# lfeng-nl/paddle-operator

Hardware: AMD Instinct MI355X
Metric: launched tokens/sec (GPT-2-medium PaddleJob through the pdo operator, collective DP over RCCL) (higher is better)
Workload: dtype bf16; 1 GPU; model=gpt2-medium, global_batch=64, micro_batch_per_gpu=64, seq_len=1024, parallelism=dp1, pod_layout=1x1, grad_reduce=bf16, buckets=2, ops=hip, device=AMD Radeon Graphics

## Files before the change

### csrc/hip/bind.cpp

```cpp
#include <c10/hip/HIPStream.h>
#include <torch/extension.h>

#include <cmath>

#include "kernels.h"

namespace {

using pdo::bf16;

hipStream_t cur_stream() { return c10::hip::getCurrentHIPStream().stream(); }

#define CHECK_DEV(t) TORCH_CHECK((t).is_cuda(), #t " must be a GPU tensor")
#define CHECK_CONTIG(t) TORCH_CHECK((t).is_contiguous(), #t " must be contiguous")
#define CHECK_BF16(t) TORCH_CHECK((t).scalar_type() == at::kBFloat16, #t " must be bf16")
#define CHECK_F32(t) TORCH_CHECK((t).scalar_type() == at::kFloat, #t " must be float32")
#define CHECK_I64(t) TORCH_CHECK((t).scalar_type() == at::kLong, #t " must be int64")
#define CHECK_IN(t) \
  CHECK_DEV(t);     \
  CHECK_CONTIG(t)
#define CHECK_RC(rc, what) TORCH_CHECK((rc) == 0, what " rejected the shape (code ", rc, ")")

inline bf16* bp(const at::Tensor& t) { return reinterpret_cast<bf16*>(t.data_ptr()); }
inline float* fp(const at::Tensor& t) { return t.data_ptr<float>(); }
// ... 324 lines not shown
                           cur_stream()), "adamw_flat");
}

void sgd_flat(at::Tensor w, at::Tensor g, at::Tensor buf, at::Tensor decay, double lr, double mom, double wd,
              double grad_scale) {
  CHECK_IN(w); CHECK_IN(g); CHECK_IN(buf); CHECK_IN(decay);
  CHECK_F32(w); CHECK_F32(g); CHECK_F32(buf); CHECK_F32(decay);
  const long long n = w.numel();
  TORCH_CHECK(g.numel() == n && buf.numel() == n && n % 1024 == 0 && decay.numel() == n / 1024);
  CHECK_RC(pdo::sgd_flat(fp(w), fp(g), fp(buf), fp(decay), n, (float)lr, (float)mom, (float)wd, (float)grad_scale,
                         cur_stream()), "sgd_flat");
}

void splitk_add(at::Tensor part, at::Tensor out, bool accumulate) {
  CHECK_IN(part); CHECK_BF16(part); CHECK_BF16(out);
  TORCH_CHECK(out.is_contiguous() && part.size(0) >= 1 && part[0].numel() == out.numel());
  CHECK_RC(pdo::splitk_add(bp(part), (int)part.size(0), out.numel(), bp(out), accumulate ? 1 : 0, cur_stream()),
           "splitk_add");
}

bool gemm_dw(at::Tensor dy, at::Tensor x, at::Tensor out, bool accumulate, int64_t splits) {
  CHECK_IN(dy); CHECK_IN(x); CHECK_IN(out); CHECK_BF16(dy); CHECK_BF16(x); CHECK_BF16(out);
  TORCH_CHECK(dy.dim() == 2 && x.dim() == 2 && dy.size(0) == x.size(0));
  const long long T = dy.size(0);
  const int M = dy.size(1), N = x.size(1);
  TORCH_CHECK(out.numel() == (int64_t)M * N, "gemm_dw: out must hold M·N elements");
  int s = pdo::gemm_dw_splits(T, M, N);
  if (s == 0) return false;
  if (splits > 0) s = (int)splits;
  at::Tensor ws;
  if (s > 1) ws = at::empty({(int64_t)s * M * N}, dy.options());
  CHECK_RC(pdo::gemm_dw(bp(dy), bp(x), T, M, N, M, N, bp(out), N, accumulate ? 1 : 0, s > 1 ? bp(ws) : nullptr, s,
                        cur_stream()), "gemm_dw");
  return true;
}

void transpose_batched(at::Tensor src, at::Tensor dst, at::Tensor table, at::Tensor host, int64_t tiles) {
  CHECK_IN(src); CHECK_IN(dst); CHECK_IN(table); CHECK_BF16(src); CHECK_BF16(dst);
  TORCH_CHECK(table.scalar_type() == at::kLong && table.dim() == 2 && table.size(1) == 5, "table: int64 [n, 5]");
  TORCH_CHECK(!host.is_cuda() && host.scalar_type() == at::kLong && host.is_contiguous() &&
              host.sizes() == table.sizes(), "transpose_batched: host table must mirror the device table");
  const at::Tensor& t = host;
  const int64_t* e = t.data_ptr<int64_t>();
  int64_t want = 0;
  for (int64_t i = 0; i < t.size(0); ++i, e += 5) {
    TORCH_CHECK(e[0] == want && e[3] % 64 == 0 && e[4] % 64 == 0 && e[3] > 0 && e[4] > 0, "transpose_batched: bad entry ", i);
    TORCH_CHECK(e[1] >= 0 && e[1] + e[3] * e[4] <= src.numel() && e[2] >= 0 && e[2] + e[3] * e[4] <= dst.numel(),
                "transpose_batched: entry ", i, " out of range");
    want += (e[3] / 64) * (e[4] / 64);
  }
  TORCH_CHECK(want == tiles, "transpose_batched: tile count mismatch");
  CHECK_RC(pdo::transpose_bf16_batched(bp(src), bp(dst), reinterpret_cast<const long long*>(table.data_ptr<int64_t>()), (int)table.size(0), tiles,
                                       cur_stream()), "transpose_batched");
}

bool gemm_nt_supported(int64_t M, int64_t N, int64_t K) {
  return M < (1LL << 31) && N < (1LL << 31) && pdo::gemm_nt_ok((int)M, (int)N, (int)K, (int)K, (int)K, (int)N);
}

static void nt_check(const at::Tensor& a, const at::Tensor& b) {
  CHECK_IN(a); CHECK_IN(b); CHECK_BF16(a); CHECK_BF16(b);
  TORCH_CHECK(a.dim() == 2 && b.dim() == 2 && a.size(1) == b.size(1), "gemm_nt: a [M, K], b [N, K]");
  TORCH_CHECK(gemm_nt_supported(a.size(0), b.size(0), a.size(1)), "gemm_nt: M, N % 256 and K % 64 required");
}

at::Tensor gemm_nt(at::Tensor a, at::Tensor b, c10::optional<at::Tensor> bias, c10::optional<at::Tensor> out) {
// ... 859 lines not shown
        py::arg("eps"), py::arg("rbias") = py::none(), py::arg("thr") = 0, py::arg("seed") = 0, py::arg("site") = 0,
        py::arg("step") = 0, py::arg("offset") = 0);
  m.def("layernorm_bwd", &layernorm_bwd, py::arg("dy"), py::arg("x"), py::arg("w"), py::arg("mean"),
        py::arg("rstd"), py::arg("grads") = py::none());
  m.def("layernorm_bwd_add", &layernorm_bwd_add, py::arg("dy"), py::arg("h"), py::arg("w"), py::arg("mean"),
        py::arg("rstd"), py::arg("dres"), py::arg("rbias"), py::arg("grads") = py::none(), py::arg("thr") = 0,
        py::arg("seed") = 0, py::arg("site") = 0, py::arg("step") = 0, py::arg("offset") = 0,
        py::arg("want_dx") = true);
  m.def("bias_gelu_fwd", &bias_gelu_fwd);
  m.def("bias_gelu_bwd", &bias_gelu_bwd, py::arg("dy"), py::arg("x"), py::arg("b"), py::arg("db_out") = py::none());
  m.def("bias_grad", &bias_grad, py::arg("dy"), py::arg("out") = py::none());
  m.def("xent_fwd", &xent_fwd);
  m.def("xent_bwd", &xent_bwd);
  m.def("xent_fused", &xent_fused);
  m.def("embed_fwd", &embed_fwd, py::arg("idx"), py::arg("wte"), py::arg("wpe"), py::arg("thr") = 0,
        py::arg("seed") = 0, py::arg("site") = 0, py::arg("step") = 0, py::arg("offset") = 0);
  m.def("embed_bwd", &embed_bwd);
  m.def("embed_bwd_sorted", &embed_bwd_sorted);
  m.def("sumsq", &sumsq);
  m.def("sumsq_chunks", &sumsq_chunks);
  m.def("set_adamw_variant", [](int v) { pdo::adamw_set_variant(v); });
  m.def("sumsq_total", &sumsq_total);
  m.def("adamw_flat", &adamw_flat);
  m.def("sgd_flat", &sgd_flat);
  m.def("splitk_add", &splitk_add);
  m.def("transpose", &transpose, py::arg("x"), py::arg("out") = py::none());
  m.def("transpose_batched", &transpose_batched);
  m.def("colsum_defer", &colsum_defer);
  m.def("colsum_flush", &colsum_flush);
  m.def("colsum_pending", &colsum_pending);
  m.def("axpy_dev_", &axpy_dev_);
  m.def("gemm_dw", &gemm_dw, py::arg("dy"), py::arg("x"), py::arg("out"), py::arg("accumulate") = true,
        py::arg("splits") = 0);
  m.def("gemm_dw_splits", &pdo::gemm_dw_splits);
  m.def("gemm_nt_supported", &gemm_nt_supported);
  m.def("gemm_nt_stats", &gemm_nt_stats);
  m.def("gemm_nt_stats_rows", [](int64_t K) { return pdo::gemm_nt_stats_rows((int)K); });
  m.def("gemm_nt_epi_ok", [](int64_t M, int64_t N, int64_t K) {
    return M < (1LL << 31) && N < (1LL << 31) && pdo::gemm_nt_epi_ok((int)M, (int)N, (int)K) != 0;
  });
  m.def("gemm_dw_impl", [](int impl) {
    const int prev = pdo::gemm_dw_get_impl();
    if (impl >= 0) pdo::gemm_dw_set_impl(impl);
    return prev;
  }, py::arg("impl") = -1, "select gemm_dw's mainloop (0 = 8-wave, 1.. = 4-wave variants); returns the previous");
  m.def("gemm_nt_impl", [](int impl) {
    const int prev = pdo::gemm_nt_get_impl();
    if (impl >= 0) pdo::gemm_nt_set_impl(impl);
    return prev;
  }, py::arg("impl") = -1, "select gemm_nt's mainloop (0 = 8-wave ring, 1 = 4-wave); returns the previous");
  m.def("gemm_nt4_dynamic", [](int on) {
    static int cur = 0;
    const int prev = cur;
    if (on >= 0) pdo::gemm_nt4_set_dynamic(cur = on);
    return prev;
  }, py::arg("on") = -1, "gemm_nt4 tile order: 1 = dynamic per-XCD counters, 0 = static (default); returns the previous");
  m.def("gemm_nt", &gemm_nt, py::arg("a"), py::arg("b"), py::arg("bias") = py::none(), py::arg("out") = py::none());
  m.def("gemm_nt_gelu", &gemm_nt_gelu, py::arg("a"), py::arg("b"), py::arg("bias"), py::arg("saved_grad") = false);
  m.def("gemm_nt_dgelu", &gemm_nt_dgelu, py::arg("a"), py::arg("b"), py::arg("pre"), py::arg("bias"),
        py::arg("db_out") = py::none(), py::arg("saved_grad") = false);
  m.def("bn_act_fwd", &bn_act_fwd);
  m.def("bn_act_bwd_pair", &bn_act_bwd_pair);
  m.def("bn_act_fwd_tiles_bnres", &bn_act_fwd_tiles_bnres);
  m.def("bn_act_fwd_tiles", &bn_act_fwd_tiles);
  m.def("conv_ok", &conv_ok);
  m.def("conv_fwd", &conv_fwd, py::arg("x"), py::arg("w"), py::arg("stride"), py::arg("pad"),
// ... 51 lines not shown
```

### csrc/hip/gemm_dw4.hip

```cpp
#include <type_traits>

#include "dw_tile.h"
#include "kernels.h"

namespace pdo {

namespace {

constexpr int BM = 256, BN = 256, BK = 64;
constexpr int LROW = 256;
constexpr int TILE = BK * LROW;
constexpr int OPB = TILE * 2;
constexpr int NTHR = 256;
using Tile = DwTile<LROW>;

__global__ __launch_bounds__(NTHR, 1) void gemm_dw4_kernel(const bf16* __restrict__ A, const bf16* __restrict__ B,
                                                           int lda, int ldb, int M, int N, int ksteps_total,
                                                           int splits, bf16* __restrict__ C, int ldc,
                                                           long long split_stride, int accumulate) {
  __shared__ __attribute__((aligned(16))) bf16 smem[2 * 2 * TILE];
  const int tid = threadIdx.x, lane = tid & 63;
  const int w = __builtin_amdgcn_readfirstlane(tid >> 6);
  const int wm = w >> 1, wn = w & 1;
  const int tiles_n = N / BN, tiles_m = (M + BM - 1) / BM;
// ... 152 lines not shown
        const int m = m0 + wm * 128 + 32 * mb + (r & 3) + 8 * (r >> 2) + 4 * hh;
        if (m >= M) continue;
        const int n = n0 + wn * 128 + 32 * nb + li;
        bf16* p = Cb + (size_t)m * ldc + n;
        float x = v[r];
        if (accumulate) x += (float)*p;
        *p = (bf16)x;
      }
    }
}

__device__ __forceinline__ int swz16(int r) { return ((r & 3) | ((((r >> 2) ^ (r >> 3)) & 1) << 2)) << 1; }
__device__ __forceinline__ int loff16(int r, int ch) { return r * LROW + ((ch ^ swz16(r)) << 3); }
__device__ __forceinline__ int frag_base16(int cb, int lane) {
  const int g = lane >> 4, t = lane & 15, q = t >> 2, p = t & 3;
  const int col = cb + 4 * p;
  return loff16(4 * g + q, col >> 3) + (col & 7);
}
template <int K0>
__device__ __forceinline__ bf16x8 frag16(const bf16* T) {
  return ld_tr8(T + K0 * LROW, T + (K0 + 16) * LROW);
}

struct DwGather {
  const bf16* x;
  unsigned xbytes;
  int C, S, IH, IW, TA, TB;
  int TC;
  float inv_TA, inv_TB;
  int st, pad;
  float* part;
};

template <bool GATHER>
__global__ __launch_bounds__(NTHR, 1) void gemm_dw4m16_kernel(const bf16* __restrict__ A, const bf16* __restrict__ B,
                                                              int lda, int ldb, int M, int N, int ksteps_total,
                                                              int splits, bf16* __restrict__ C, int ldc,
                                                              long long split_stride, int accumulate,
                                                              const DwGather gx) {
  __shared__ __attribute__((aligned(16))) bf16 smem[2 * 2 * TILE];
  const int tid = threadIdx.x, lane = tid & 63;
  const int w = __builtin_amdgcn_readfirstlane(tid >> 6);
  const int wm = w >> 1, wn = w & 1;
  const int tiles_n = N / BN, tiles_m = (M + BM - 1) / BM;
  const int nwg = tiles_m * tiles_n * splits;
  const int id = xcd_remap((int)blockIdx.x, nwg);
  const int tn = id % tiles_n;
  const int tm = (id / tiles_n) % tiles_m;
  const int split = id / (tiles_n * tiles_m);
  const int pq = (ksteps_total >> 1) / splits, pr = (ksteps_total >> 1) % splits;
  const int k0 = 2 * (split * pq + min(split, pr));
  const int nk = 2 * (pq + (split < pr ? 1 : 0));
  const int m0 = tm * BM, n0 = tn * BN;

  const int rl = lane >> 5, rw = 2 * w + rl;
  unsigned voffA[2], voffB[2];
#pragma unroll
  for (int par = 0; par < 2; ++par) {
    const int cs = (lane & 31) ^ swz16(8 * par + rw);
    const int csa = (m0 + BM > M && cs >= 16) ? cs - 16 : cs;
    voffA[par] = (unsigned)((rl * lda + csa * 8) * 2);
    voffB[par] = (unsigned)((rl * ldb + cs * 8) * 2);
  }
  const bf16* baseA = A + ((size_t)k0 * BK + 2 * w) * lda + m0;
  const bf16* baseB = GATHER ? A : B + ((size_t)k0 * BK + 2 * w) * ldb + n0;
  const unsigned stepAb = (unsigned)(16 * lda), stepBb = (unsigned)(16 * ldb);
  const unsigned lds0 = lds_addr(smem) + (unsigned)(w * 1024);
  int gdh[2] = {0, 0}, gdw[2] = {0, 0}, gci[2] = {0, 0};
  const __amdgpu_buffer_rsrc_t rsX = buf_rsrc(GATHER ? gx.x : A, GATHER ? (int)gx.xbytes : 0);
  if constexpr (GATHER) {
#pragma unroll
    for (int par = 0; par < 2; ++par) {
      const int col = n0 + (((lane & 31) ^ swz16(8 * par + rw)) << 3);
      const int tap = col / gx.C, r = tap / gx.S;
      gci[par] = col - tap * gx.C;
      gdh[par] = col < gx.TC ? r - gx.pad : -(1 << 20);
      gdw[par] = tap - r * gx.S - gx.pad;
    }
  }
  struct Src {
    const char* a;
    const char* b;
    unsigned sa, sb;
    int kt;
  };
// ... 42 lines not shown
  bf16x8 f0[16], f1[16];

  {
    const Src s0 = srcs(0), s1 = srcs(1);
#pragma unroll
    for (int p = 0; p < 16; ++p) dma(s0, B0{}, p);
#pragma unroll
    for (int p = 0; p < 16; ++p) dma(s1, B1{}, p);
  }
  vm_wait<16>();
  __builtin_amdgcn_sched_barrier(0);
  __builtin_amdgcn_s_barrier();
  __builtin_amdgcn_sched_barrier(0);
#pragma unroll
  for (int q = 0; q < 16; ++q) f0[q] = rd(B0{}, 0, q);
  auto tileH = [&](int t, auto buf_tag, auto more_tag, auto first_tag, auto eout_tag) {
    constexpr int BUF = decltype(buf_tag)::value;
    constexpr bool MORE = decltype(more_tag)::value;
    constexpr bool FIRST = decltype(first_tag)::value;
    constexpr bool EOUT = decltype(eout_tag)::value;
    using NB = std::integral_constant<int, BUF ^ 1>;
    using SB = std::integral_constant<int, BUF>;
    Src sn2{};
    if constexpr (EOUT) sn2 = srcs(t + 2);
    asm volatile("s_waitcnt lgkmcnt(0)" ::: "memory");
    __builtin_amdgcn_sched_barrier(0);
    __builtin_amdgcn_s_barrier();
    __builtin_amdgcn_sched_barrier(0);
#pragma unroll
    for (int g = 0; g < 16; ++g) {
      const int mb = g >> 1, nb0 = 4 * (g & 1);
#pragma unroll
      for (int u = 0; u < 4; ++u) {
        if (FIRST) mfma16_acc0(acc[mb][nb0 + u], f0[mb], f0[8 + nb0 + u]);
        else mfma16_acc(acc[mb][nb0 + u], f0[mb], f0[8 + nb0 + u]);
      }
      f1[g] = rd(buf_tag, 1, g);
      if constexpr (EOUT) {
        if (g & 1) dma(sn2, SB{}, (g >> 1) < 4 ? (g >> 1) : (g >> 1) + 4);
      }
      __builtin_amdgcn_sched_barrier(0);
    }
    if constexpr (MORE || EOUT) {
      if constexpr (EOUT)
        asm volatile("s_waitcnt vmcnt(8) lgkmcnt(0)" ::: "memory");
      else
        asm volatile("s_waitcnt vmcnt(0) lgkmcnt(0)" ::: "memory");
      __builtin_amdgcn_sched_barrier(0);
      __builtin_amdgcn_s_barrier();
      __builtin_amdgcn_sched_barrier(0);
    }
#pragma unroll
    for (int g = 0; g < 16; ++g) {
      const int mb = g >> 1, nb0 = 4 * (g & 1);
#pragma unroll
      for (int u = 0; u < 4; ++u) mfma16_acc(acc[mb][nb0 + u], f1[mb], f1[8 + nb0 + u]);
      if constexpr (MORE) f0[g] = rd(NB{}, 0, g);
      if constexpr (EOUT) {
        if (g & 1) dma(sn2, SB{}, (g >> 1) < 4 ? (g >> 1) + 4 : (g >> 1) + 8);
      }
      __builtin_amdgcn_sched_barrier(0);
    }
  };
  using T_ = std::true_type;
  using F_ = std::false_type;
  tileH(0, B0{}, T_{}, T_{}, T_{});
  tileH(1, B1{}, T_{}, F_{}, T_{});
  for (int t = 2; t < nk - 2; t += 2) {
    tileH(t, B0{}, T_{}, F_{}, T_{});
    tileH(t + 1, B1{}, T_{}, F_{}, T_{});
  }
  tileH(nk - 2, B0{}, T_{}, F_{}, F_{});
  tileH(nk - 1, B1{}, F_{}, F_{}, F_{});

  asm volatile("s_nop 7\n\ts_nop 7" ::: "memory");
  bf16* Cb = C + (size_t)split * split_stride;
  const int g4 = lane >> 4, li = lane & 15;
  if (m0 + wm * 128 >= M) return;
  if constexpr (GATHER) {
    float* P = gx.part + (size_t)split * split_stride;
#pragma unroll
    for (int mb = 0; mb < 8; ++mb)
#pragma unroll
      for (int nb = 0; nb < 8; ++nb) {
        float v[4];
#pragma unroll
        for (int r = 0; r < 4; ++r) asm volatile("v_accvgpr_read_b32 %0, %1" : "=v"(v[r]) : "a"(acc[mb][nb][r]));
#pragma unroll
        for (int r = 0; r < 4; ++r) {
          const int m = m0 + wm * 128 + 16 * mb + 4 * g4 + r;
          P[(size_t)m * ldc + n0 + wn * 128 + 16 * nb + li] = v[r];
        }
      }
    return;
  }
#pragma unroll
  for (int mb = 0; mb < 8; ++mb)
#pragma unroll
    for (int nb = 0; nb < 8; ++nb) {
      float v[4];
#pragma unroll
      for (int r = 0; r < 4; ++r) asm volatile("v_accvgpr_read_b32 %0, %1" : "=v"(v[r]) : "a"(acc[mb][nb][r]));
#pragma unroll
      for (int r = 0; r < 4; ++r) {
        const int m = m0 + wm * 128 + 16 * mb + 4 * g4 + r;
        bf16* p = Cb + (size_t)m * ldc + n0 + wn * 128 + 16 * nb + li;
        float x = v[r];
        if (accumulate) x += (float)*p;
        *p = (bf16)x;
      }
    }
}

}

int gemm_dw4(const bf16* A, const bf16* B, long long T, int M, int N, int lda, int ldb, bf16* C, int ldc,
             int accumulate, bf16* ws, int splits, hipStream_t st, int variant) {
  if (M % (BM / 2) || N % BN || T % BK || splits < 1 || splits > 16) return -2;
  const long long ks = T / BK;
  if (ks > 0x7fffffffLL) return -2;
  if (ks % 2 || (ks / 2) / splits < 2) return -2;
  const int tiles = ((M + BM - 1) / BM) * (N / BN);
  const int grid = tiles * splits;
  bf16* out = C;
  int ldo = ldc;
  long long stride = 0;
  int acc = accumulate;
  if (splits > 1) {
    if (!ws || ldc != N) return -3;
    out = ws;
    ldo = N;
    stride = (long long)M * N;
    acc = 0;
  }
  if (variant == 1)
    gemm_dw4_kernel<<<grid, NTHR, 0, st>>>(A, B, lda, ldb, M, N, (int)ks, splits, out, ldo, stride, acc);
  else
    gemm_dw4m16_kernel<false><<<grid, NTHR, 0, st>>>(A, B, lda, ldb, M, N, (int)ks, splits, out, ldo, stride, acc,
                                                     DwGather{});
  if (splits > 1) return splitk_add(ws, splits, (long long)M * N, C, accumulate, st);
  return 0;
}

int conv_wgrad_dw4_splits(int Kout, int TC, long long M) {
  const long long tiles = (long long)((Kout + 255) / 256) * ((TC + 255) / 256);
  const long long pairs = M / 128;
  static const int ncu = [] {
    int dev = 0, n = 0;
    if (hipGetDevice(&dev) != hipSuccess || hipDeviceGetAttribute(&n, hipDeviceAttributeMultiprocessorCount, dev) != hipSuccess)
      n = 256;
    return n > 0 ? n : 256;
  }();
  long long sp = ncu / tiles;
  if (sp > pairs / 2) sp = pairs / 2;
  if (sp > 256) sp = 256;
  return sp < 1 ? 1 : (int)sp;
}

int conv_wgrad_dw4(const bf16* dy, const bf16* x, int N, int H, int W, int C, int Kout, int R, int S, int stride,
                   int pad, float* part, int splits, hipStream_t st) {
  const int Ho = (H + 2 * pad - R) / stride + 1, Wo = (W + 2 * pad - S) / stride + 1;
  const long long M = (long long)N * Ho * Wo;
  const int TC = R * S * C, TCp = (TC + BN - 1) / BN * BN;
  if (Kout % (BM / 2) || C % 8 || M % (2 * BK) || M >= (1LL << 31)) return -2;
  const long long ks = M / BK;
  if (splits < 1 || (ks / 2) / splits < 2) return -2;
  if ((long long)N * H * W * C * 2 >= (1LL << 31)) return -2;
  DwGather g{x, (unsigned)((long long)N * H * W * C * 2), C, S, H, W, Ho, Wo, TC, 1.f / (float)Ho, 1.f / (float)Wo,
             stride, pad, part};
  const int grid = ((Kout + BM - 1) / BM) * (TCp / BN) * splits;
  gemm_dw4m16_kernel<true><<<grid, NTHR, 0, st>>>(dy, nullptr, Kout, 0, Kout, TCp, (int)ks, splits, nullptr, TCp,
                                                  (long long)Kout * TCp, 0, g);
  return 0;
}

}
```

### csrc/hip/kernels.h

```cpp
#pragma once
#include <hip/hip_runtime.h>
#include <stdint.h>

#include "philox.h"

namespace pdo {
typedef __bf16 bf16;

struct ColOut {
  bf16* p[3] = {nullptr, nullptr, nullptr};
  int seg = 1 << 30;
  int acc = 0;
  static ColOut one(bf16* o, int C) {
    ColOut c;
    c.p[0] = o;
    c.seg = C;
    return c;
  }
};

int layernorm_fwd(const bf16* x, const bf16* r, const bf16* rb, const bf16* w, const bf16* b, bf16* h, bf16* y,
                  float* mean, float* rstd, int N, int C, float eps, hipStream_t st,
                  const DropArgs* drop = nullptr);
int layernorm_bwd_grid(int N);
// ... 68 lines not shown
                       float* ss, const float* rtile_part, int rG, int rtile_rows, const bf16* r, const float* rw,
                       const float* rb, float* rrunning_mean, float* rrunning_var, float reps, float rmomentum,
                       float* rmean, float* rinvstd, float* rss, long long M, int C, int relu, bf16* y,
                       unsigned char* mask, hipStream_t st, float* merge = nullptr);
int bn_fwd_scratch_floats(long long M, int C);
int bn_bwd_scratch_pair_floats(long long M, int C);
int bn_bwd_pair(const bf16* dy, const unsigned char* mask, const bf16* x, const float* mean, const float* invstd,
                const float* w, float* dw, float* db, int accumulate, const bf16* r, const float* rmean,
                const float* rinvstd, const float* rw, float* rdw, float* rdb, int raccumulate, long long M, int C,
                bf16* dx, bf16* dr, float* scratch, hipStream_t st);
int bn_relu_pool_fwd_tiles(const float* tile_part, int G, int tile_rows, const bf16* x, const float* w, const float* b,
                           float* running_mean, float* running_var, int N, int H, int W, int C, float eps,
                           float momentum, bf16* y, uint8_t* arg, bf16* xsel, float* mean, float* invstd, float* ss,
                           hipStream_t st, float* merge = nullptr);
int pool_bn_bwd_scratch_floats(int N, int H, int W, int C);
int pool_bn_bwd(const bf16* dy, const bf16* y, const bf16* xsel, const uint8_t* arg, const bf16* x, const float* mean,
                const float* invstd, const float* w, const float* b, int N, int H, int W, int C, bf16* dx, float* dw,
                float* db, int accumulate, float* scratch, hipStream_t st);
int bn_fwd(const bf16* x, const bf16* res, const float* w, const float* b, float* running_mean, float* running_var,
           long long M, int C, float eps, float momentum, int relu, bf16* y, float* mean, float* invstd,
           float* scratch, hipStream_t st, unsigned char* mask = nullptr);
int bn_bwd_scratch_floats(long long M, int C);
int bn_bwd(const bf16* dy, const bf16* y, const bf16* x, const float* mean, const float* invstd, const float* w,
           const float* b, long long M, int C, int relu, bf16* dx, bf16* dres, float* dw, float* db, int accumulate,
           float* scratch, hipStream_t st);
int maxpool3s2_fwd(const bf16* x, int N, int H, int W, int C, bf16* y, uint8_t* arg, hipStream_t st);
int maxpool3s2_bwd(const bf16* dy, const uint8_t* arg, int N, int H, int W, int C, bf16* dx, hipStream_t st);
int gap_bwd(const bf16* dy, int N, int HW, int C, bf16* dx, hipStream_t st);
int gemm_dw_splits(long long T, int M, int N);
int gemm_dw(const bf16* A, const bf16* B, long long T, int M, int N, int lda, int ldb, bf16* C, int ldc,
            int accumulate, bf16* ws, int splits, hipStream_t st);
int gemm_dw4(const bf16* A, const bf16* B, long long T, int M, int N, int lda, int ldb, bf16* C, int ldc,
             int accumulate, bf16* ws, int splits, hipStream_t st, int variant);
void gemm_dw_set_impl(int impl);
int gemm_dw_get_impl();
int gemm_nt_ok(int M, int N, int K, int lda, int ldb, int ldc);
int gemm_nt_epi_ok(int M, int N, int K);
int gemm_nt_stats_rows(int K);
int gemm_nt_dbias_rows(int M, int K);
int gemm_nt(const bf16* A, const bf16* B, int M, int N, int K, int lda, int ldb, bf16* C, int ldc, int epi,
            const bf16* bias, bf16* Y, int ldy, float* dbias_part, hipStream_t st);
int gemm_nt4(const bf16* A, const bf16* B, int M, int N, int K, int lda, int ldb, bf16* C, int ldc, int epi,
             const bf16* bias, bf16* Y, int ldy, float* dbias_part, hipStream_t st);
void gemm_nt_set_impl(int impl);
void gemm_nt4_set_dynamic(int on);
int gemm_nt_get_impl();
int transpose_bf16(const bf16* in, bf16* out, int R, int C, hipStream_t st);
int transpose_bf16_batched(const bf16* src, bf16* dst, const long long* table, int n, long long tiles,
                           hipStream_t st);
int splitk_add(const bf16* part, int s, long long n, bf16* out, int accumulate, hipStream_t st);

int bias_gelu_fwd(const bf16* x, const bf16* b, bf16* y, long long N, int F, hipStream_t st);
int bias_gelu_bwd_groups(long long N, int F);
int bias_gelu_bwd(const bf16* dy, const bf16* x, const bf16* b, bf16* dx, float* part, float* scratch, bf16* db,
                  long long N, int F, hipStream_t st, int accumulate = 0);

int xent_fwd(const bf16* logits, const int64_t* tgt, float* row_loss, float* lse, float* stats, int N, int Vp, int V,
             hipStream_t st);
int xent_fused(bf16* logits, const int64_t* tgt, const float* inv_cnt, float* row_loss, float* loss, int N, int Vp,
               int V, hipStream_t st);
int xent_bwd(const bf16* logits, const int64_t* tgt, const float* lse, const float* dloss, const float* stats,
             bf16* dlogits, int N, int Vp, int V, hipStream_t st);

int embed_fwd(const int64_t* idx, const bf16* wte, const bf16* wpe, bf16* y, int B, int S, int C, hipStream_t st,
              const DropArgs* drop = nullptr);
int embed_bwd(const bf16* dy, const int64_t* idx, float* acc, bf16* dwte, bf16* dwpe, int B, int S, int C, int Vp,
// ... 41 lines not shown
```

### paddle_operator_amd/ops/__init__.py

```python
from .core import (
    _HIP_DW, _NT_ALL, _arena_grads, _direct_ok, _fwd_gemm, _input_grad, _signal_ready, _splitk, _weight_grad,
    _weight_grad_lib, _workspace, deferred_reductions, flush_deferred, linear, ref_attention, ref_bias_gelu,
    ref_cross_entropy, ref_layer_norm, transpose, use_hip,
    Dropout, dropout_spec, dropout_thr, philox4x32_10, philox_keep_mask, ref_dropout,
    ATTN_SITE0, attn_dropout_spec, attn_dropout_thr, philox_attn_keep_mask)
from .gpt2 import (
    _LMHeadXentFn, _LM_CHUNK, _QKV_FUSED, _RES_EPI, _XENT_FUSED, _NT_GELU, _NT_DGELU, _NT_GD, add_layer_norm,
    attention, bias_gelu, cross_entropy, embedding, layer_norm, layer_norm_res, linear_add_layer_norm, lm_head_xent, mlp, mlp_add_layer_norm,
    qkv_attention)
from .resnet import (
    _BNActBNResFn, _BNLink, _BNReluPoolFn, _CompactGradLink, _ResMaskLink, _StemFn, _BN_FUSED, _DS_FUSED,
    _GEMM_BN_STATS, _BN_LINK, _BN_LINK_USED, _DS_COMPACT, _DS_COMPACT_USED, _HIP_CONV, _HIP_STEM, _RES_MASK,
    _RES_MASK_USED, _STEM_POOL, _apply_bitmask, _stem_ok, bn_act, conv1x1, conv_bn_act, conv_bn_ds_act,
    conv_bn_relu_maxpool, global_avg_pool,
    max_pool_3x3s2)

__all__ = [
    "layer_norm", "layer_norm_res", "add_layer_norm", "bias_gelu", "attention", "cross_entropy",
    "embedding", "ref_layer_norm", "ref_bias_gelu", "ref_attention",
    "ref_cross_entropy", "use_hip", "linear", "mlp", "qkv_attention", "lm_head_xent",
    "conv_bn_act", "conv_bn_ds_act", "bn_act", "deferred_reductions",
    "Dropout", "dropout_spec", "philox_keep_mask", "attn_dropout_spec", "philox_attn_keep_mask", "ATTN_SITE0",
]
```

### paddle_operator_amd/ops/core.py

```python
from __future__ import annotations

import math
import os

import torch
import torch.nn.functional as F

from .. import _native


def use_hip(t: torch.Tensor) -> bool:
    if not t.is_cuda:
        return False
    if _native.ops_mode() == "torch":
        return False
    _native.require_hip()
    return True


def ref_layer_norm(x, w, b, eps=1e-5):
    y = F.layer_norm(x.float(), (x.shape[-1],), w.float(), b.float(), eps)
    return y.to(x.dtype)


# ... 228 lines not shown
    return (w.is_cuda and w.dtype == torch.bfloat16 and w.dim() == 2 and w.shape[0] % 64 == 0
            and w.shape[1] % 64 == 0 and w.is_contiguous())


def transpose(w, out=None):
    if out is None:
        wt = _live_wt(w)
        if wt is not None:
            return wt
    if _transposable(w):
        if out is not None:
            return _native.require_hip().transpose(w, out)
        return _native.require_hip().transpose(w)
    return w.t().contiguous()


def _weight_grad(w, dy2, x2):
    Fo, K = dy2.shape[1], x2.shape[1]
    if not _direct_ok(w):
        if (_HIP_DW[0] and dy2.is_cuda and dy2.dtype == torch.bfloat16 and dy2.is_contiguous()
                and x2.is_contiguous()):
            g = torch.empty(Fo, K, device=dy2.device, dtype=dy2.dtype)
            if _native.require_hip().gemm_dw(dy2, x2, g, False):
                return g
        s = _splitk(dy2.shape[0], Fo, K) if use_hip(dy2) else 1
        if s == 1:
            return dy2.t() @ x2
        T = dy2.shape[0] // s
        part = torch.bmm(dy2.view(s, T, Fo).transpose(1, 2), x2.view(s, T, K),
                         out=_workspace(dy2.device, s * Fo * K).view(s, Fo, K))
        g = torch.empty(Fo, K, device=dy2.device, dtype=dy2.dtype)
        _native.require_hip().splitk_add(part, g, False)
        return g
    if not (_HIP_DW[0] and dy2.is_cuda and w.grad.dtype == torch.bfloat16 and dy2.is_contiguous()
            and x2.is_contiguous() and _native.require_hip().gemm_dw(dy2, x2, w.grad, True)):
        _weight_grad_lib(w, dy2, x2)
    w._pdo_ready(w)
    return None


_HIP_DW = [True]


def _weight_grad_lib(w, dy2, x2):
    Fo, K = dy2.shape[1], x2.shape[1]
    g = w.grad.view(Fo, K)
    s = _splitk(dy2.shape[0], Fo, K)
    if s > 1:
        T = dy2.shape[0] // s
        part = torch.bmm(dy2.view(s, T, Fo).transpose(1, 2), x2.view(s, T, K),
                         out=_workspace(dy2.device, s * Fo * K).view(s, Fo, K))
        _native.require_hip().splitk_add(part, g, True)
    else:
        g.addmm_(dy2.t(), x2)


def _direct_ok(p) -> bool:
    g = p.grad
    return (getattr(p, "_pdo_direct", False) and g is not None and g.is_contiguous()
            and torch.is_grad_enabled() is False)


def _arena_grads(params):
    out = []
    for p in params:
        if p is None or not _direct_ok(p) or p.grad.dtype != torch.bfloat16:
            return None
        out.append(p.grad.view(-1))
    return out


class deferred_reductions:

    def __init__(self, device):
        self.on = torch.device(device).type == "cuda" and _native.ops_mode() != "torch"
        self.prev = False

    def __enter__(self):
        if self.on:
            self.prev = _native.require_hip().colsum_defer(True)
        return self

    def __exit__(self, *exc):
        if self.on:
            _native.require_hip().colsum_defer(self.prev)


def flush_deferred():
    m = _native.hip_ext()
    if m is not None and m.colsum_pending():
        m.colsum_flush()


def _signal_ready(params):
    for p in params:
        p._pdo_ready(p)


def linear(x, w, b=None):
    if use_hip(x):
        return _LinearFn.apply(x, w, b)
    return F.linear(x, w, b)
```

### paddle_operator_amd/train.py

```python
from __future__ import annotations

import contextlib
import os
import time
from dataclasses import dataclass

import torch
import torch.distributed as dist

from .models.gpt2 import GPT2, GPT2Config
from .ops import deferred_reductions
from .ops.optim import FlatAdamW, cosine_lr
from .parallel.ddp import BucketedDDP
from .parallel.flat import FlatParams
from .utils import trace
from .utils.topology import bucket_bytes_for


@dataclass
class DistInfo:
    rank: int = 0
    world: int = 1
    local_rank: int = 0

    @property
    def is_main(self):
        return self.rank == 0


def init_distributed(backend: str | None = None, timeout_s: int = 600) -> DistInfo:
    world = int(os.environ.get("WORLD_SIZE", "1"))
    rank = int(os.environ.get("RANK", "0"))
    local = int(os.environ.get("LOCAL_RANK", str(rank)))
    info = DistInfo(rank, world, local)
    backend = backend or os.environ.get("PDO_DIST_BACKEND") or None
    if torch.cuda.is_available():
        ndev = torch.cuda.device_count()
        if backend == "gloo" and local >= ndev:
            local = local % ndev
            info.local_rank = local
        torch.cuda.set_device(local)
    if backend is None:
        backend = "nccl" if torch.cuda.is_available() else "gloo"
    if (world > 1 or backend == "nccl") and not dist.is_initialized():
# ... 77 lines not shown
            self.val = TokenStream(val_data, self.B, self.S, cfg.vocab_size, self.device, data_seed, EVAL_STREAM,
                                   rank, data_device_gb)
        self.acc = torch.zeros(self.flat.grads.numel(), dtype=torch.float32, device=self.device) if self.K > 2 else None

    def sync_initial_weights(self):
        self.ddp.broadcast_params(0)
        self.opt.master.copy_(self.flat.params.float())

    def batch(self):
        if self.data is not None:
            return self.data.batch(self.data_step)
        V = self.cfg.vocab_size
        idx = torch.randint(0, V, (self.B, self.S + 1), device=self.device, generator=self.gen)
        return idx[:, :-1], idx[:, 1:]

    def next_lr(self) -> float:
        if self.lr_schedule == "cosine":
            return cosine_lr(self.opt.step_count, self.opt.lr, self.lr_warmup, self.lr_decay_steps, self.lr_min_ratio)
        return self.opt.lr

    def step(self, idx=None, tgt=None):
        if self.K > 1:
            return self._step_accum(idx, tgt)
        if idx is None:
            idx, tgt = self.batch()
        self.model.drop_step = self.drop_step & 0xFFFFFFFF
        self.drop_step += 1
        self.data_step += 1
        self.flat.zero_grad()
        self.ddp.prepare()
        with self.flat.wt_scope():
            with trace.range("forward"):
                loss = self.model(idx, tgt)
            with trace.range("backward"), deferred_reductions(self.device):
                loss.backward()
        with trace.range("allreduce_drain"):
            self.ddp.finish(self.opt if self.opt.max_grad_norm else None)
        with trace.range("optimizer"):
            self.opt.step(grad_scale=self.ddp.grad_scale, lr=self.next_lr())
        return loss

    def _step_accum(self, idx, tgt):
        K, B = self.K, self.B
        if idx is not None and idx.shape[0] != K * B:
            raise ValueError(f"step(idx, tgt) with grad_accum={K} takes {K * B} rows, got {idx.shape[0]}")
        losses = []
        self.flat.zero_grad()
        with self.flat.wt_scope():
            for i in range(1, K + 1):
                x, y = (idx[(i - 1) * B:i * B], tgt[(i - 1) * B:i * B]) if idx is not None else self.batch()
                self.model.drop_step = self.drop_step & 0xFFFFFFFF
                self.drop_step += 1
                self.data_step += 1
                self.ddp.prepare()
                with contextlib.nullcontext() if i == K else self.ddp.no_sync():
                    with trace.range("forward"):
                        loss = self.model(x, y)
                    with trace.range("backward"), deferred_reductions(self.device):
                        (loss * (1.0 / K)).backward()
                    with trace.range("allreduce_drain"):
                        self.ddp.finish(self.opt if self.opt.max_grad_norm and i == K else None)
                losses.append(loss.detach())
                if self.acc is not None and _ACCUM_FP32[0] and i < K:
                    self._fold(init=(i == 1), emit=(i == K - 1))
        with trace.range("optimizer"):
            self.opt.step(grad_scale=self.ddp.grad_scale, lr=self.next_lr())
        return torch.stack(losses).mean()

    def _fold(self, init: bool, emit: bool):
        g = self.flat.grads
        if g.is_cuda and g.dtype == torch.bfloat16:
            from . import _native
            _native.require_hip().grad_accum_fold(g, self.acc, init, emit)
            return
        if init:
            self.acc.zero_()
        self.acc.add_(g.float())
        if emit:
            g.copy_(self.acc)
        else:
            g.zero_()

    @torch.no_grad()
    def evaluate(self, n_batches: int) -> float:
        if self.val is None:
            raise RuntimeError("evaluate() needs val_data")
        was_training = self.model.training
        self.model.eval()
        try:
            tot = torch.zeros(2, dtype=torch.float64, device=self.device)
            for m in range(n_batches):
# ... 45 lines not shown
```

Before: 464,400 tokens/s.

## Batch weight-gradient GEMMs into grouped launches to fill CUs

Queues weight-gradient GEMMs during backward and launches them together as one grouped dw kernel. A tile table maps blocks to problems, and the queue flushes when the total tile count is a multiple of the CU count. The grouped path swaps the MFMA operand order so the epilogue writes bf16x4 vectors. The aim is to remove wave-quantization tail waste and per-launch overhead for medium GPT-2 weight GEMMs without split-K. In exchange it delays gradient readiness signals, which can hurt overlap with the DDP allreduce, and it keeps activations alive longer.

```diff
diff --git a/csrc/hip/bind.cpp b/csrc/hip/bind.cpp
--- a/csrc/hip/bind.cpp
+++ b/csrc/hip/bind.cpp
@@ -380,6 +380,48 @@
   if (s > 1) ws = at::empty({(int64_t)s * M * N}, dy.options());
   CHECK_RC(pdo::gemm_dw(bp(dy), bp(x), T, M, N, M, N, bp(out), N, accumulate ? 1 : 0, s > 1 ? bp(ws) : nullptr, s,
                         cur_stream()), "gemm_dw");
+  return true;
+}
+
+bool gemm_dw_grouped(std::vector<at::Tensor> dys, std::vector<at::Tensor> xs, std::vector<at::Tensor> outs,
+                     std::vector<bool> accumulates) {
+  const size_t n = dys.size();
+  TORCH_CHECK(xs.size() == n && outs.size() == n && accumulates.size() == n, "gemm_dw_grouped: list lengths differ");
+  auto rows2d = [](const at::Tensor& t) {
+    return t.dim() == 2 && t.size(0) > 0 && t.size(1) > 0 && t.stride(1) == 1 && t.stride(0) >= t.size(1) &&
+           t.stride(0) < (1LL << 24);
+  };
+  std::vector<pdo::DwProblem> ps(n);
+  for (size_t i = 0; i < n; ++i) {
+    const at::Tensor &dy = dys[i], &x = xs[i], &out = outs[i];
+    CHECK_DEV(dy); CHECK_DEV(x); CHECK_DEV(out); CHECK_BF16(dy); CHECK_BF16(x); CHECK_BF16(out);
+    TORCH_CHECK(dy.device() == out.device() && x.device() == out.device(), "gemm_dw_grouped: operands on different devices");
+    TORCH_CHECK(dy.dim() == 2 && x.dim() == 2 && out.dim() == 2 && dy.size(0) == x.size(0) &&
+                out.size(0) == dy.size(1) && out.size(1) == x.size(1), "gemm_dw_grouped: out must be [M, N] of dy [T, M], x [T, N]");
+    if (!rows2d(dy) || !rows2d(x) || !rows2d(out)) return false;
+    auto al16 = [](const at::Tensor& t) { return (uintptr_t)t.data_ptr() % 16 == 0 && t.stride(0) % 8 == 0; };
+    if (!al16(dy) || !al16(x)) return false;
+    const long long T = dy.size(0);
+    if (dy.size(1) >= (1LL << 31) || x.size(1) >= (1LL << 31)) return false;
+    const int M = (int)dy.size(1), N = (int)x.size(1);
+    if (!pdo::gemm_dw4_grouped_ok(T, M, N)) return false;
+    ps[i] = pdo::DwProblem{bp(dy), bp(x), bp(out), T, M, N, (int)dy.stride(0), (int)x.stride(0), (int)out.stride(0),
+                           accumulates[i] ? 1 : 0};
+  }
+  auto overlap = [](const pdo::DwProblem& a, const pdo::DwProblem& b) {
+    const bf16* ae = a.C + (size_t)(a.M - 1) * a.ldc + a.N;
+    const bf16* be = b.C + (size_t)(b.M - 1) * b.ldc + b.N;
+    return a.C < be && b.C < ae;
+  };
+  size_t i0 = 0;
+  for (size_t i = 0; i <= n; ++i) {
+    bool cut = i == n;
+    for (size_t k = i0; k < i && !cut; ++k) cut = overlap(ps[k], ps[i]);
+    if (cut && i > i0) {
+      CHECK_RC(pdo::gemm_dw4_grouped(ps.data() + i0, (int)(i - i0), cur_stream()), "gemm_dw_grouped");
+      i0 = i;
+    }
+  }
   return true;
 }
 
@@ -1305,6 +1347,8 @@
   m.def("axpy_dev_", &axpy_dev_);
   m.def("gemm_dw", &gemm_dw, py::arg("dy"), py::arg("x"), py::arg("out"), py::arg("accumulate") = true,
         py::arg("splits") = 0);
+  m.def("gemm_dw_grouped", &gemm_dw_grouped, py::arg("dys"), py::arg("xs"), py::arg("outs"), py::arg("accumulates"));
+  m.def("gemm_dw_grouped_ok", &pdo::gemm_dw4_grouped_ok);
   m.def("gemm_dw_splits", &pdo::gemm_dw_splits);
   m.def("gemm_nt_supported", &gemm_nt_supported);
   m.def("gemm_nt_stats", &gemm_nt_stats);
diff --git a/csrc/hip/gemm_dw4.hip b/csrc/hip/gemm_dw4.hip
--- a/csrc/hip/gemm_dw4.hip
+++ b/csrc/hip/gemm_dw4.hip
@@ -208,25 +208,72 @@
   float* part;
 };
 
-template <bool GATHER>
-__global__ __launch_bounds__(NTHR, 1) void gemm_dw4m16_kernel(const bf16* __restrict__ A, const bf16* __restrict__ B,
-                                                              int lda, int ldb, int M, int N, int ksteps_total,
-                                                              int splits, bf16* __restrict__ C, int ldc,
-                                                              long long split_stride, int accumulate,
-                                                              const DwGather gx) {
+struct DwGroupEntry {
+  const bf16* A;
+  const bf16* B;
+  bf16* C;
+  int lda, ldb, ldc, M, N, ksteps, accumulate;
+};
+struct DwGroupTable {
+  int n;
+  int first[DW_GROUP_MAX + 1];
+  DwGroupEntry p[DW_GROUP_MAX];
+};
+struct DwNoGroup {};
+
+__device__ __forceinline__ int dw_group_tile(int b, int total) {
+  const int full = total & ~255;
+  if (b < full) return (b & ~255) + ((b & 7) << 5) + ((b >> 3) & 31);
+  return full + xcd_remap(b - full, total - full);
+}
+__device__ __forceinline__ void dw_group_mn(int t, int tiles_m, int tiles_n, int& tm, int& tn) {
+  const int fulls = tiles_n >> 2, per = 4 * tiles_m;
+  if (t < fulls * per) {
+    const int s = t / per, r = t - s * per;
+    tm = r >> 2;
+    tn = 4 * s + (r & 3);
+  } else {
+    const int r = t - fulls * per, wd = tiles_n & 3;
+    tm = r / wd;
+    tn = 4 * fulls + r - tm * wd;
+  }
+}
+
+template <bool GATHER, bool GROUPED>
+__global__ __launch_bounds__(NTHR, 1) void gemm_dw4m16_kernel(
+    const bf16* __restrict__ A_, const bf16* __restrict__ B_, int lda_, int ldb_, int M_, int N_, int ksteps_total,
+    int splits, bf16* __restrict__ C_, int ldc_, long long split_stride, int accumulate_, const DwGather gx,
+    const std::conditional_t<GROUPED, DwGroupTable, DwNoGroup> tb) {
   __shared__ __attribute__((aligned(16))) bf16 smem[2 * 2 * TILE];
+  constexpr bool SWAP = GROUPED;
   const int tid = threadIdx.x, lane = tid & 63;
   const int w = __builtin_amdgcn_readfirstlane(tid >> 6);
   const int wm = w >> 1, wn = w & 1;
-  const int tiles_n = N / BN, tiles_m = (M + BM - 1) / BM;
-  const int nwg = tiles_m * tiles_n * splits;
-  const int id = xcd_remap((int)blockIdx.x, nwg);
-  const int tn = id % tiles_n;
-  const int tm = (id / tiles_n) % tiles_m;
-  const int split = id / (tiles_n * tiles_m);
-  const int pq = (ksteps_total >> 1) / splits, pr = (ksteps_total >> 1) % splits;
-  const int k0 = 2 * (split * pq + min(split, pr));
-  const int nk = 2 * (pq + (split < pr ? 1 : 0));
+  const bf16* A = A_;
+  const bf16* B = B_;
+  bf16* C = C_;
+  int lda = lda_, ldb = ldb_, ldc = ldc_, M = M_, N = N_, accumulate = accumulate_;
+  int tm, tn, split, k0, nk;
+  if constexpr (GROUPED) {
+    const int g = dw_group_tile((int)blockIdx.x, tb.first[tb.n]);
+    int pi = 0;
+    while (g >= tb.first[pi + 1]) ++pi;
+    const DwGroupEntry& e = tb.p[pi];
+    A = e.A, B = e.B, C = e.C;
+    lda = e.lda, ldb = e.ldb, ldc = e.ldc, M = e.M, N = e.N, accumulate = e.accumulate;
+    dw_group_mn(g - tb.first[pi], (M + BM - 1) / BM, N / BN, tm, tn);
+    split = 0, k0 = 0, nk = e.ksteps;
+  } else {
+    const int tiles_n = N / BN, tiles_m = (M + BM - 1) / BM;
+    const int nwg = tiles_m * tiles_n * splits;
+    const int id = xcd_remap((int)blockIdx.x, nwg);
+    tn = id % tiles_n;
+    tm = (id / tiles_n) % tiles_m;
+    split = id / (tiles_n * tiles_m);
+    const int pq = (ksteps_total >> 1) / splits, pr = (ksteps_total >> 1) % splits;
+    k0 = 2 * (split * pq + min(split, pr));
+    nk = 2 * (pq + (split < pr ? 1 : 0));
+  }
   const int m0 = tm * BM, n0 = tn * BN;
 
   const int rl = lane >> 5, rw = 2 * w + rl;
@@ -335,8 +382,10 @@
       const int mb = g >> 1, nb0 = 4 * (g & 1);
 #pragma unroll
       for (int u = 0; u < 4; ++u) {
-        if (FIRST) mfma16_acc0(acc[mb][nb0 + u], f0[mb], f0[8 + nb0 + u]);
-        else mfma16_acc(acc[mb][nb0 + u], f0[mb], f0[8 + nb0 + u]);
+        const bf16x8& fr = f0[SWAP ? 8 + nb0 + u : mb];
+        const bf16x8& fc = f0[SWAP ? mb : 8 + nb0 + u];
+        if (FIRST) mfma16_acc0(acc[mb][nb0 + u], fr, fc);
+        else mfma16_acc(acc[mb][nb0 + u], fr, fc);
       }
       f1[g] = rd(buf_tag, 1, g);
       if constexpr (EOUT) {
@@ -357,7 +406,8 @@
     for (int g = 0; g < 16; ++g) {
       const int mb = g >> 1, nb0 = 4 * (g & 1);
 #pragma unroll
-      for (int u = 0; u < 4; ++u) mfma16_acc(acc[mb][nb0 + u], f1[mb], f1[8 + nb0 + u]);
+      for (int u = 0; u < 4; ++u)
+        mfma16_acc(acc[mb][nb0 + u], f1[SWAP ? 8 + nb0 + u : mb], f1[SWAP ? mb : 8 + nb0 + u]);
       if constexpr (MORE) f0[g] = rd(NB{}, 0, g);
       if constexpr (EOUT) {
         if (g & 1) dma(sn2, SB{}, (g >> 1) < 4 ? (g >> 1) + 4 : (g >> 1) + 8);
@@ -397,6 +447,26 @@
       }
     return;
   }
+  if constexpr (!SWAP) {
+#pragma unroll
+    for (int mb = 0; mb < 8; ++mb)
+#pragma unroll
+      for (int nb = 0; nb < 8; ++nb) {
+        float v[4];
+#pragma unroll
+        for (int r = 0; r < 4; ++r) asm volatile("v_accvgpr_read_b32 %0, %1" : "=v"(v[r]) : "a"(acc[mb][nb][r]));
+#pragma unroll
+        for (int r = 0; r < 4; ++r) {
+          const int m = m0 + wm * 128 + 16 * mb + 4 * g4 + r;
+          bf16* p = Cb + (size_t)m * ldc + n0 + wn * 128 + 16 * nb + li;
+          float x = v[r];
+          if (accumulate) x += (float)*p;
+          *p = (bf16)x;
+        }
+      }
+    return;
+  }
+  const bool al8 = ((reinterpret_cast<size_t>(Cb) | ((size_t)ldc * 2)) & 7) == 0;
 #pragma unroll
   for (int mb = 0; mb < 8; ++mb)
 #pragma unroll
@@ -404,13 +474,26 @@
       float v[4];
 #pragma unroll
       for (int r = 0; r < 4; ++r) asm volatile("v_accvgpr_read_b32 %0, %1" : "=v"(v[r]) : "a"(acc[mb][nb][r]));
-#pragma unroll
-      for (int r = 0; r < 4; ++r) {
-        const int m = m0 + wm * 128 + 16 * mb + 4 * g4 + r;
-        bf16* p = Cb + (size_t)m * ldc + n0 + wn * 128 + 16 * nb + li;
-        float x = v[r];
-        if (accumulate) x += (float)*p;
-        *p = (bf16)x;
+      const int m = m0 + wm * 128 + 16 * mb + li;
+      bf16* q = Cb + (size_t)m * ldc + n0 + wn * 128 + 16 * nb + 4 * g4;
+      if (al8) {
+        bf16x4* p = reinterpret_cast<bf16x4*>(q);
+        if (accumulate) {
+          const bf16x4 o = *p;
+#pragma unroll
+          for (int r = 0; r < 4; ++r) v[r] += (float)o[r];
+        }
+        bf16x4 y;
+#pragma unroll
+        for (int r = 0; r < 4; ++r) y[r] = (bf16)v[r];
+        *p = y;
+      } else {
+#pragma unroll
+        for (int r = 0; r < 4; ++r) {
+          float x = v[r];
+          if (accumulate) x += (float)q[r];
+          q[r] = (bf16)x;
+        }
       }
     }
 }
@@ -439,9 +522,44 @@
   if (variant == 1)
     gemm_dw4_kernel<<<grid, NTHR, 0, st>>>(A, B, lda, ldb, M, N, (int)ks, splits, out, ldo, stride, acc);
   else
-    gemm_dw4m16_kernel<false><<<grid, NTHR, 0, st>>>(A, B, lda, ldb, M, N, (int)ks, splits, out, ldo, stride, acc,
-                                                     DwGather{});
+    gemm_dw4m16_kernel<false, false><<<grid, NTHR, 0, st>>>(A, B, lda, ldb, M, N, (int)ks, splits, out, ldo, stride,
+                                                            acc, DwGather{}, DwNoGroup{});
   if (splits > 1) return splitk_add(ws, splits, (long long)M * N, C, accumulate, st);
+  return 0;
+}
+
+bool gemm_dw4_grouped_ok(long long T, int M, int N) {
+  return M > 0 && N > 0 && M % (BM / 2) == 0 && N % BN == 0 && T % (2 * BK) == 0 && T >= 4 * BK &&
+         T / BK <= 0x7fffffffLL;
+}
+
+int gemm_dw4_grouped(const DwProblem* probs, int n, hipStream_t st) {
+  if (n < 0) return -2;
+  for (int i = 0; i < n; ++i) {
+    const DwProblem& q = probs[i];
+    if (!gemm_dw4_grouped_ok(q.T, q.M, q.N) || q.lda < q.M || q.ldb < q.N || q.ldc < q.N || !q.A || !q.B || !q.C)
+      return -2;
+    if ((long long)q.lda * 16 * 8 >= (1LL << 31) || (long long)q.ldb * 16 * 8 >= (1LL << 31)) return -2;
+  }
+  for (int i0 = 0; i0 < n;) {
+    DwGroupTable tb;
+    tb.n = 0;
+    tb.first[0] = 0;
+    while (i0 < n && tb.n < DW_GROUP_MAX) {
+      const DwProblem& q = probs[i0];
+      const long long tiles = (long long)((q.M + BM - 1) / BM) * (q.N / BN);
+      if (tb.first[tb.n] + tiles > (1 << 24)) {
+        if (tb.n == 0) return -2;
+        break;
+      }
+      tb.p[tb.n] = DwGroupEntry{q.A, q.B, q.C, q.lda, q.ldb, q.ldc, q.M, q.N, (int)(q.T / BK), q.accumulate};
+      tb.first[tb.n + 1] = tb.first[tb.n] + (int)tiles;
+      ++tb.n;
+      ++i0;
+    }
+    gemm_dw4m16_kernel<false, true><<<tb.first[tb.n], NTHR, 0, st>>>(nullptr, nullptr, 0, 0, 0, 0, 0, 1, nullptr, 0, 0,
+                                                                    0, DwGather{}, tb);
+  }
   return 0;
 }
 
@@ -472,8 +590,8 @@
   DwGather g{x, (unsigned)((long long)N * H * W * C * 2), C, S, H, W, Ho, Wo, TC, 1.f / (float)Ho, 1.f / (float)Wo,
              stride, pad, part};
   const int grid = ((Kout + BM - 1) / BM) * (TCp / BN) * splits;
-  gemm_dw4m16_kernel<true><<<grid, NTHR, 0, st>>>(dy, nullptr, Kout, 0, Kout, TCp, (int)ks, splits, nullptr, TCp,
-                                                  (long long)Kout * TCp, 0, g);
+  gemm_dw4m16_kernel<true, false><<<grid, NTHR, 0, st>>>(dy, nullptr, Kout, 0, Kout, TCp, (int)ks, splits, nullptr,
+                                                         TCp, (long long)Kout * TCp, 0, g, DwNoGroup{});
   return 0;
 }
 
diff --git a/csrc/hip/kernels.h b/csrc/hip/kernels.h
--- a/csrc/hip/kernels.h
+++ b/csrc/hip/kernels.h
@@ -124,6 +124,16 @@
             int accumulate, bf16* ws, int splits, hipStream_t st);
 int gemm_dw4(const bf16* A, const bf16* B, long long T, int M, int N, int lda, int ldb, bf16* C, int ldc,
              int accumulate, bf16* ws, int splits, hipStream_t st, int variant);
+constexpr int DW_GROUP_MAX = 32;
+struct DwProblem {
+  const bf16* A;
+  const bf16* B;
+  bf16* C;
+  long long T;
+  int M, N, lda, ldb, ldc, accumulate;
+};
+bool gemm_dw4_grouped_ok(long long T, int M, int N);
+int gemm_dw4_grouped(const DwProblem* probs, int n, hipStream_t st);
 void gemm_dw_set_impl(int impl);
 int gemm_dw_get_impl();
 int gemm_nt_ok(int M, int N, int K, int lda, int ldb, int ldc);
diff --git a/paddle_operator_amd/ops/__init__.py b/paddle_operator_amd/ops/__init__.py
--- a/paddle_operator_amd/ops/__init__.py
+++ b/paddle_operator_amd/ops/__init__.py
@@ -1,6 +1,8 @@
 from .core import (
     _HIP_DW, _NT_ALL, _arena_grads, _direct_ok, _fwd_gemm, _input_grad, _signal_ready, _splitk, _weight_grad,
     _weight_grad_lib, _workspace, deferred_reductions, flush_deferred, linear, ref_attention, ref_bias_gelu,
+    _DW_GROUPED, _DW_CUS, _DW_CAP_BYTES, deferred_weight_grads, flush_weight_grads, dw_tiles, dw_should_flush,
+    dw_grouped_prefix,
     ref_cross_entropy, ref_layer_norm, transpose, use_hip,
     Dropout, dropout_spec, dropout_thr, philox4x32_10, philox_keep_mask, ref_dropout,
     ATTN_SITE0, attn_dropout_spec, attn_dropout_thr, philox_attn_keep_mask)
@@ -20,5 +22,6 @@
     "embedding", "ref_layer_norm", "ref_bias_gelu", "ref_attention",
     "ref_cross_entropy", "use_hip", "linear", "mlp", "qkv_attention", "lm_head_xent",
     "conv_bn_act", "conv_bn_ds_act", "bn_act", "deferred_reductions",
+    "deferred_weight_grads", "flush_weight_grads",
     "Dropout", "dropout_spec", "philox_keep_mask", "attn_dropout_spec", "philox_attn_keep_mask", "ATTN_SITE0",
 ]
diff --git a/paddle_operator_amd/ops/core.py b/paddle_operator_amd/ops/core.py
--- a/paddle_operator_amd/ops/core.py
+++ b/paddle_operator_amd/ops/core.py
@@ -284,11 +284,17 @@
         g = torch.empty(Fo, K, device=dy2.device, dtype=dy2.dtype)
         _native.require_hip().splitk_add(part, g, False)
         return g
+    if _dw_queue.push(w, dy2, x2):
+        return None
+    _weight_grad_now(w, dy2, x2)
+    w._pdo_ready(w)
+    return None
+
+
+def _weight_grad_now(w, dy2, x2):
     if not (_HIP_DW[0] and dy2.is_cuda and w.grad.dtype == torch.bfloat16 and dy2.is_contiguous()
             and x2.is_contiguous() and _native.require_hip().gemm_dw(dy2, x2, w.grad, True)):
         _weight_grad_lib(w, dy2, x2)
-    w._pdo_ready(w)
-    return None
 
 
 _HIP_DW = [True]
@@ -339,9 +345,111 @@
 
 
 def flush_deferred():
+    flush_weight_grads()
     m = _native.hip_ext()
     if m is not None and m.colsum_pending():
         m.colsum_flush()
+
+
+_DW_GROUPED = [True]
+_DW_CUS = [0]
+_DW_CAP_BYTES = [16 << 30]
+_DW_MIN_ROUNDS = 3
+_DW_FILL = 0.94
+
+
+def dw_tiles(M: int, N: int) -> int:
+    return ((M + 255) // 256) * (N // 256)
+
+
+def dw_should_flush(tiles, held_bytes: int, cus: int, cap_bytes: int, min_rounds: int = _DW_MIN_ROUNDS) -> bool:
+    total = sum(tiles)
+    if total > 0 and total % cus == 0 and total >= min_rounds * cus:
+        return True
+    return held_bytes > cap_bytes
+
+
+def dw_grouped_prefix(tiles, cus: int, fill: float = _DW_FILL) -> int:
+    best, total = 0, 0
+    for i, t in enumerate(tiles):
+        total += t
+        last = total % cus or cus
+        if total > 0 and last >= fill * cus:
+            best = i + 1
+    return best
+
+
+class _DWQueue:
+    def __init__(self):
+        self.depth = 0
+        self.entries = []
+        self.tiles = []
+        self.held = 0
+        self.cus = 0
+        self.n_grouped = 0
+
+    def push(self, w, dy2, x2) -> bool:
+        if not (self.depth and _DW_GROUPED[0] and _HIP_DW[0] and dy2.is_cuda and dy2.dtype == torch.bfloat16
+                and x2.dtype == torch.bfloat16 and w.grad.dtype == torch.bfloat16 and dy2.is_contiguous()
+                and x2.is_contiguous() and dy2.dim() == 2 and x2.dim() == 2):
+            return False
+        T, M, N = dy2.shape[0], dy2.shape[1], x2.shape[1]
+        if x2.shape[0] != T or w.grad.numel() != M * N:
+            return False
+        if not _native.require_hip().gemm_dw_grouped_ok(T, M, N):
+            return False
+        if not self.cus:
+            self.cus = _DW_CUS[0] or torch.cuda.get_device_properties(dy2.device).multi_processor_count
+        self.entries.append((w, dy2, x2))
+        self.tiles.append(dw_tiles(M, N))
+        self.held += (dy2.numel() + x2.numel()) * 2
+        if dw_should_flush(self.tiles, self.held, self.cus, _DW_CAP_BYTES[0]):
+            self.flush()
+        return True
+
+    def flush(self):
+        if not self.entries:
+            return
+        entries, tiles, cus = self.entries, self.tiles, self.cus
+        self.entries, self.tiles, self.held, self.cus = [], [], 0, 0
+        k = dw_grouped_prefix(tiles, cus)
+        if k:
+            m = _native.require_hip()
+            outs = [w.grad.view(dy2.shape[1], x2.shape[1]) for w, dy2, x2 in entries[:k]]
+            if not m.gemm_dw_grouped([e[1] for e in entries[:k]], [e[2] for e in entries[:k]], outs, [True] * k):
+                raise RuntimeError("gemm_dw_grouped rejected a queued weight gradient")
+            self.n_grouped += k
+        for w, dy2, x2 in entries[k:]:
+            _weight_grad_now(w, dy2, x2)
+        for w, _, _ in entries:
+            w._pdo_ready(w)
+
+
+_dw_queue = _DWQueue()
+
+
+class deferred_weight_grads:
+
+    def __init__(self, device):
+        self.on = torch.device(device).type == "cuda" and _native.ops_mode() != "torch"
+
+    def __enter__(self):
+        if self.on:
+            _dw_queue.depth += 1
+        return self
+
+    def __exit__(self, *exc):
+        if self.on:
+            _dw_queue.depth -= 1
+            if _dw_queue.depth == 0:
+                if exc and exc[0] is not None:
+                    _dw_queue.entries, _dw_queue.tiles, _dw_queue.held = [], [], 0
+                else:
+                    _dw_queue.flush()
+
+
+def flush_weight_grads():
+    _dw_queue.flush()
 
 
 def _signal_ready(params):
diff --git a/paddle_operator_amd/train.py b/paddle_operator_amd/train.py
--- a/paddle_operator_amd/train.py
+++ b/paddle_operator_amd/train.py
@@ -9,7 +9,7 @@
 import torch.distributed as dist
 
 from .models.gpt2 import GPT2, GPT2Config
-from .ops import deferred_reductions
+from .ops import deferred_reductions, deferred_weight_grads
 from .ops.optim import FlatAdamW, cosine_lr
 from .parallel.ddp import BucketedDDP
 from .parallel.flat import FlatParams
@@ -153,7 +153,7 @@
         with self.flat.wt_scope():
             with trace.range("forward"):
                 loss = self.model(idx, tgt)
-            with trace.range("backward"), deferred_reductions(self.device):
+            with trace.range("backward"), deferred_reductions(self.device), deferred_weight_grads(self.device):
                 loss.backward()
         with trace.range("allreduce_drain"):
             self.ddp.finish(self.opt if self.opt.max_grad_norm else None)
@@ -177,7 +177,8 @@
                 with contextlib.nullcontext() if i == K else self.ddp.no_sync():
                     with trace.range("forward"):
                         loss = self.model(x, y)
-                    with trace.range("backward"), deferred_reductions(self.device):
+                    with trace.range("backward"), deferred_reductions(self.device), \
+                            deferred_weight_grads(self.device):
                         (loss * (1.0 / K)).backward()
                     with trace.range("allreduce_drain"):
                         self.ddp.finish(self.opt if self.opt.max_grad_norm and i == K else None)
```

Measured after the change: 469,600 tokens/s (median of 6 runs). +1.1%, better.
